# dpeerlab/segger

Hardware: AMD Instinct MI355X
Metric: edges scored/sec (tx->cell) fwd+bwd (higher is better)
Workload: dtype bf16; 1 GPU; C2: single Xenium-scale tile per GPU, 1000000 tx, 10000 nuclei, k=15 kNN (Ett=15000000, Etb=393796, Ep=2435646), training step fwd+bwd+Adam, attention dropout 0.2; parallelism=dp1

## Files before the change

### include/segger_amd.h

```cpp
#ifndef SEGGER_AMD_H
#define SEGGER_AMD_H

#include <stddef.h>
#include <stdint.h>

#ifdef __cplusplus
extern "C" {
#endif

#if defined(__GNUC__) || defined(__clang__)
#pragma GCC visibility push(default)
#endif

#define SEGGER_ABI_VERSION 30

enum segger_status {
  SEGGER_OK = 0,
  SEGGER_EINVAL = -1,
  SEGGER_EUNSUPPORTED = -2,
  SEGGER_EHIP = -3,
  SEGGER_EWORKSPACE = -4
};

enum segger_dtype { SEGGER_F32 = 0, SEGGER_BF16 = 1, SEGGER_F16 = 2 };

typedef void* segger_stream_t;

int segger_abi_version(void);
const char* segger_last_error(void);
// ... 85 lines not shown
  int64_t ld_gxr;
  float* grad_att;
  float* grad_bias;
  void* workspace;
  size_t workspace_bytes;
  const uint8_t* keep_bits_dst;
  const uint8_t* keep_bits_src;
  int32_t src_unique;
  void* zero_rows_out;
  int64_t ld_zero;
  int32_t grad_xl_zeroed;
  int32_t passes;
} segger_gatv2_bwd_args;

size_t segger_gatv2_bwd_workspace_bytes(int64_t n_dst, int32_t heads, int32_t channels);
int segger_gatv2_bwd(const segger_gatv2_bwd_args* args, segger_stream_t stream);
int segger_gatv2_bwd_pair(const segger_gatv2_bwd_args* a, const segger_gatv2_bwd_args* b, segger_stream_t stream);
int segger_dropout_bits(const int32_t* eid, int64_t n_edges, int32_t heads, float dropout_p, const uint64_t* seeds,
                        int32_t n_seeds, const uint64_t* seed_dev, uint8_t* bits, int64_t plane_stride,
                        segger_stream_t stream);
typedef struct segger_bits_job {
  const int32_t* eid;
  int64_t n_edges;
  const uint64_t* seeds;
  int32_t n_seeds;
  int32_t reserved_;
  uint8_t* bits;
  int64_t plane_stride;
} segger_bits_job;
int segger_dropout_bits_many(const segger_bits_job* jobs, int32_t n_jobs, int32_t heads, float dropout_p,
// ... 338 lines not shown
```

### segger_amd/_lib.py

```python
from __future__ import annotations

import ctypes as C
import os
from typing import Optional

import torch

_HERE = os.path.dirname(os.path.abspath(__file__))
LIB_PATH = os.environ.get("SEGGER_AMD_LIB") or os.path.join(_HERE, "libsegger_amd.so")
ABI_VERSION = 30

SEGGER_F32, SEGGER_BF16, SEGGER_F16 = 0, 1, 2
DTYPE_CODE = {torch.float32: SEGGER_F32, torch.bfloat16: SEGGER_BF16, torch.float16: SEGGER_F16}


class SeggerAmdError(RuntimeError):
    pass


c_i64p = C.c_void_p
vp = C.c_void_p


class Csr(C.Structure):
    _fields_ = [("indptr", vp), ("col", vp), ("eid", vp),
# ... 173 lines not shown
class WgradArgs(C.Structure):
    _fields_ = [("dy", vp), ("ld_dy", C.c_int64), ("x", vp), ("ld_x", C.c_int64), ("w_t", vp), ("n_rows", C.c_int64),
                ("m_out", C.c_int32), ("reserved_", C.c_int32), ("grad_w", vp), ("grad_b", vp), ("dx", vp),
                ("ld_dx", C.c_int64), ("workspace", vp), ("workspace_bytes", C.c_size_t)]


EXPORTS = {
    "segger_abi_version": (C.c_int, []),
    "segger_csr_block_tables": (C.c_int, [vp, vp, vp, C.c_int64, C.c_int64, vp, vp, vp, vp, vp]),
    "segger_last_error": (C.c_char_p, []),
    "segger_csr_from_coo_workspace_bytes": (C.c_size_t, [C.c_int64, C.c_int64]),
    "segger_csr_from_coo": (C.c_int, [vp, vp, C.c_int64, C.c_int64, C.c_int64, vp, vp, vp, vp, vp, C.c_size_t, vp]),
    "segger_csr_row_order": (C.c_int, [vp, C.c_int64, C.c_int32, vp, vp]),
    "segger_gatv2_fwd": (C.c_int, [C.POINTER(GatFwdArgs), vp]),
    "segger_gatv2_bwd_workspace_bytes": (C.c_size_t, [C.c_int64, C.c_int32, C.c_int32]),
    "segger_gatv2_bwd": (C.c_int, [C.POINTER(GatBwdArgs), vp]),
    "segger_dropout_bits": (C.c_int, [vp, C.c_int64, C.c_int32, C.c_float, vp, C.c_int32, vp, vp, C.c_int64, vp]),
    "segger_gatv2_has_specialised": (C.c_int, [C.c_int32, C.c_int32]),
    "segger_coo_unique": (C.c_int, [vp, C.c_int64, C.c_int64, vp, vp, vp]),
    "segger_stage": (C.c_int, [C.POINTER(StageSeg), C.c_int32, vp]),
    "segger_adam_step": (C.c_int, [C.POINTER(AdamTensor), C.c_int32, C.c_double, C.c_double, C.c_double, C.c_double, vp]),
    "segger_adam_step_ex": (C.c_int, [C.POINTER(AdamTensor), C.c_int32, C.c_double, C.c_double, C.c_double, C.c_double, C.c_int32, vp, C.c_int64, vp]),
    "segger_adam_step_dev": (C.c_int, [C.POINTER(AdamTensor), C.c_int32, vp, C.c_int32, vp, C.c_int64, vp]),
    "segger_transpose_many": (C.c_int, [C.POINTER(TransposeSeg), C.c_int32, vp]),
    "segger_posmlp_supported": (C.c_int, [C.c_int32, C.c_int32, C.c_int32]),
    "segger_posmlp_fwd": (C.c_int, [vp, vp, vp, vp, C.c_int64, C.c_float, C.c_float, vp, vp, vp, vp, vp, vp, vp, vp, vp,
                                    C.c_int32, C.c_int32, vp]),
    "segger_posmlp_wgrad": (C.c_int, [vp, C.c_int64, vp, C.c_int64, C.c_float, C.c_int32, vp, vp, vp, C.c_size_t, vp]),
    "segger_sample_negatives": (C.c_int, [vp, C.c_int64, C.c_int64, vp, C.c_uint64, vp, vp, vp]),
    "segger_edge_cos_argmax": (C.c_int, [C.POINTER(EdgeArgmaxArgs), vp]),
# ... 158 lines not shown
```

### segger_amd/csrc/gatv2.hip

```cpp
#include "gatv2_launch.h"
#include "draws.h"

namespace segger {

constexpr int kSlabSplits = 128;

__global__ __launch_bounds__(256) void slab_reduce_stage1(const float* __restrict__ slab, int64_t nblocks, int width,
                                                         float* __restrict__ part) {
  __shared__ float sm[4][64];
  const int lane = threadIdx.x & 63, wave = threadIdx.x >> 6;
  const int colx = blockIdx.x * 64 + lane;
  const int64_t per = (nblocks + kSlabSplits - 1) / kSlabSplits;
  const int64_t r0 = (int64_t)blockIdx.y * per;
  const int64_t r1 = r0 + per < nblocks ? r0 + per : nblocks;
  float s = 0.f;
  if (colx < width)
    for (int64_t r = r0 + wave; r < r1; r += 4) s += slab[r * width + colx];
  sm[wave][lane] = s;
  __syncthreads();
  if (wave == 0 && colx < width) part[(int64_t)blockIdx.y * width + colx] = sm[0][lane] + sm[1][lane] + sm[2][lane] + sm[3][lane];
}

__global__ __launch_bounds__(256) void slab_reduce_stage2(const float* __restrict__ part, int width, int hc,
                                                         float* __restrict__ grad_att, float* __restrict__ grad_bias) {
  const int colx = blockIdx.x * 256 + threadIdx.x;
  if (colx >= width) return;
  float t = 0.f;
  for (int r = 0; r < kSlabSplits; ++r) t += part[(int64_t)r * width + colx];
  if (colx < hc) grad_att[colx] = t;
  else if (grad_bias) grad_bias[colx - hc] = t;
}

__global__ __launch_bounds__(256) void zero_rows_kernel(char* __restrict__ base, int64_t pitch, int64_t pieces, int64_t total) {
  const int64_t i = (int64_t)blockIdx.x * 256 + threadIdx.x;
  if (i >= total) return;
  *reinterpret_cast<u32x4*>(base + (i / pieces) * pitch + (i % pieces) * 16) = u32x4{0u, 0u, 0u, 0u};
}

__global__ __launch_bounds__(256) void dropout_bits_kernel(BitsParams p) { dropout_bits_body(p, blockIdx.x); }
__global__ __launch_bounds__(256) void dropout_bits_many_kernel(BitsJobs j) { dropout_bits_body(j.job[blockIdx.y], blockIdx.x); }

namespace {

constexpr double kWavePerRowDegree = 32.0;

// ... 114 lines not shown
                   use_wave_per_row(b->by_dst) && !a->alpha && !b->alpha;
  if (!one) {
    if (!ea) CHECK_RC(launch(Pass::Fwd, pa, a->dtype, a->heads, a->channels, use_wave_per_row(a->by_dst), (hipStream_t)stream));
    if (!eb) CHECK_RC(launch(Pass::Fwd, pb, b->dtype, b->heads, b->channels, use_wave_per_row(b->by_dst), (hipStream_t)stream));
    return SEGGER_OK;
  }
  switch (a->dtype) {
    case SEGGER_F32:  return gatv2_launch_fwd_pair_f32(pa, pb, a->heads, a->channels, (hipStream_t)stream);
    case SEGGER_BF16: return gatv2_launch_fwd_pair_bf16(pa, pb, a->heads, a->channels, (hipStream_t)stream);
    case SEGGER_F16:  return gatv2_launch_fwd_pair_f16(pa, pb, a->heads, a->channels, (hipStream_t)stream);
  }
  set_error("gatv2: unknown dtype %d", a->dtype);
  return SEGGER_EINVAL;
}

extern "C" size_t segger_gatv2_bwd_workspace_bytes(int64_t n_dst, int32_t heads, int32_t channels) {
  if (n_dst <= 0 || heads <= 0 || channels <= 0) return 16;
  const int64_t per = 4 * (int64_t)bwd_row_iters(n_dst);
  const int64_t blocks = (n_dst + per - 1) / per + kNumXcd;
  return (size_t)(blocks + kSlabSplits) * 2 * heads * channels * sizeof(float);
}

namespace {
struct BwdState {
  GatParams p;
  bool direct = false, specialised = false;
  int64_t n_dst = 0, n_src = 0, n_edges = 0;
};

int bwd_prepare(const segger_gatv2_bwd_args* a, BwdState& s) {
  SEGGER_REQUIRE(a != nullptr, "segger_gatv2_bwd: args is NULL");
  SEGGER_REQUIRE(a->heads > 0 && a->channels > 0, "segger_gatv2_bwd: heads/channels must be positive");
  const int hc = a->heads * a->channels;
  const bool specialised = gatv2_has_specialised(a->heads, a->channels);
  g_need_align = specialised;
// ... 12 lines not shown
  if (n_dst > 0) {
    CHECK_RC(check_rows("x_r", a->x_r, a->ld_xr, a->dtype, hc));
    CHECK_RC(check_rows("grad_out", a->grad_out, a->ld_go, a->dtype, hc));
    CHECK_RC(check_rows("pre", a->pre, a->ld_pre, a->dtype, hc));
    CHECK_RC(check_rows("grad_pre", a->grad_pre, a->ld_gp, a->dtype, hc));
    CHECK_RC(check_rows("grad_xr", a->grad_xr, a->ld_gxr, a->dtype, hc));
    SEGGER_REQUIRE(a->lse && a->dsum, "segger_gatv2_bwd: lse / dsum is NULL");
  }
  if (n_src > 0) {
    CHECK_RC(check_rows("x_l", a->x_l, a->ld_xl, a->dtype, hc));
    CHECK_RC(check_rows("grad_xl", a->grad_xl, a->ld_gxl, a->dtype, hc));
  }
  SEGGER_REQUIRE(!(a->dropout_p > 0.f) || n_edges == 0 ||
                     ((a->by_dst.eid || a->keep_bits_dst) && (direct || a->by_src.eid || a->keep_bits_src)),
                 "segger_gatv2_bwd: eid arrays (or keep_bits) are required for dropout");
  const size_t need = segger_gatv2_bwd_workspace_bytes(n_dst, a->heads, a->channels);
  if (a->workspace == nullptr || a->workspace_bytes < need) {
    set_error("segger_gatv2_bwd: workspace %zu < %zu bytes", a->workspace_bytes, need);
    return SEGGER_EWORKSPACE;
  }
  SEGGER_REQUIRE(!a->zero_rows_out || (!direct && specialised),
                 "segger_gatv2_bwd: zero_rows_out needs the two-pass backward of a specialised geometry");
  if (a->zero_rows_out && n_src > 0) CHECK_RC(check_rows("zero_rows_out", a->zero_rows_out, a->ld_zero, a->dtype, hc));

  s.direct = direct; s.specialised = specialised; s.n_dst = n_dst; s.n_src = n_src; s.n_edges = n_edges;
  GatParams& p = s.p;
  p = GatParams{};
  p.xl = a->x_l; p.ld_xl = a->ld_xl; p.xr = a->x_r; p.ld_xr = a->ld_xr;
  p.att = a->att; p.bias = a->bias;
  p.pre = const_cast<void*>(a->pre); p.ld_pre = a->ld_pre; p.lse = const_cast<float*>(a->lse);
  p.gout = a->grad_out; p.ld_go = a->ld_go; p.gpre = a->grad_pre; p.ld_gp = a->ld_gp; p.dsum = a->dsum;
// ... 6 lines not shown

void bwd_dst_params(const segger_gatv2_bwd_args* a, BwdState& s) {
  GatParams& p = s.p;
  p.indptr = a->by_dst.indptr; p.col = a->by_dst.col; p.eid = a->by_dst.eid; p.order = a->by_dst.row_order;
  p.n_rows = s.n_dst; p.n_edges = s.n_edges; p.rows_per_wave_iter = bwd_row_iters(s.n_dst);
  p.bits = a->keep_bits_dst;
  p.direct_gxl = s.direct ? 1 : 0;
  p.zero_rows = nullptr; p.ld_zero = 0;
}

void bwd_src_params(const segger_gatv2_bwd_args* a, BwdState& s) {
  GatParams& p = s.p;
  p.direct_gxl = 0;
  p.indptr = a->by_src.indptr; p.col = a->by_src.col; p.eid = a->by_src.eid; p.order = a->by_src.row_order;
  p.bits = a->keep_bits_src;
  p.n_rows = s.n_src; p.rows_per_wave_iter = 1;
  p.zero_rows = a->zero_rows_out; p.ld_zero = a->ld_zero;
}

int bwd_zero_fill(const segger_gatv2_bwd_args* a, const BwdState& s, hipStream_t stream) {
  const size_t es = elem_size(a->dtype);
  const int64_t pieces = (int64_t)a->heads * a->channels * es / 16, total = s.n_src * pieces;
  hipLaunchKernelGGL(zero_rows_kernel, dim3((unsigned)((total + 255) / 256)), dim3(256), 0, stream,
                     static_cast<char*>(a->grad_xl), (int64_t)a->ld_gxl * (int64_t)es, pieces, total);
  SEGGER_LAUNCH_CHECK("zero_rows_kernel");
  return SEGGER_OK;
}

int bwd_reduce_slab(const segger_gatv2_bwd_args* a, const BwdState& s, hipStream_t stream) {
  if (!s.specialised) return SEGGER_OK;
  const GatParams& p = s.p;
  const int hc = a->heads * a->channels, width = 2 * hc;
  float* part = p.slab + p.nblocks * width;
  if (defer_reduce(ReduceSeg{p.slab, p.nblocks, width, hc, a->grad_att, a->grad_bias, part}, stream)) return SEGGER_OK;
  hipLaunchKernelGGL(slab_reduce_stage1, dim3((width + 63) / 64, kSlabSplits), dim3(256), 0, stream,
                     p.slab, p.nblocks, width, part);
  hipLaunchKernelGGL(slab_reduce_stage2, dim3((width + 255) / 256), dim3(256), 0, stream,
                     part, width, hc, a->grad_att, a->grad_bias);
  SEGGER_LAUNCH_CHECK("slab_reduce kernels");
  return SEGGER_OK;
}

int bwd_no_destinations(const segger_gatv2_bwd_args* a, hipStream_t stream) {
  const int hc = a->heads * a->channels;
  SEGGER_HIP(hipMemsetAsync(a->grad_att, 0, hc * sizeof(float), stream));
  if (a->grad_bias) SEGGER_HIP(hipMemsetAsync(a->grad_bias, 0, hc * sizeof(float), stream));
  return SEGGER_OK;
}

int64_t bwd_pair_max_rows() {
  static const int64_t v = [] {
    const char* e = getenv("SEGGER_BWD_PAIR_MAX_ROWS");
    return e ? (int64_t)atoll(e) : (int64_t)SEGGER_BWD_PAIR_MAX_ROWS;
  }();
  return v;
}
}

extern "C" int segger_gatv2_bwd(const segger_gatv2_bwd_args* a, segger_stream_t stream_) {
  hipStream_t stream = (hipStream_t)stream_;
  BwdState s;
  CHECK_RC(bwd_prepare(a, s));
  SEGGER_REQUIRE(a->passes >= 0 && a->passes <= 3, "segger_gatv2_bwd: passes must be 0 (both), 1 (destination), 2 (source) or 3");
  if (a->passes != 2) {
    bwd_dst_params(a, s);
    if (s.direct && s.n_src > 0 && !a->grad_xl_zeroed) CHECK_RC(bwd_zero_fill(a, s, stream));
    if (s.n_dst > 0) {
      GenericOut gen; gen.grad_att = a->grad_att; gen.grad_bias = a->grad_bias;
      CHECK_RC(launch(Pass::BwdDst, s.p, a->dtype, a->heads, a->channels, use_wave_per_row(a->by_dst), stream, gen));
      if (a->passes != 3) CHECK_RC(bwd_reduce_slab(a, s, stream));
    } else {
      CHECK_RC(bwd_no_destinations(a, stream));
    }
  }
  if (s.direct || a->passes == 1 || a->passes == 3) return SEGGER_OK;
  bwd_src_params(a, s);
  if (s.n_src > 0) CHECK_RC(launch(Pass::BwdSrc, s.p, a->dtype, a->heads, a->channels, use_wave_per_row(a->by_src), stream));
  return SEGGER_OK;
}

extern "C" int segger_gatv2_bwd_pair(const segger_gatv2_bwd_args* a, const segger_gatv2_bwd_args* b, segger_stream_t stream_) {
  hipStream_t stream = (hipStream_t)stream_;
  BwdState sa, sb;
  CHECK_RC(bwd_prepare(a, sa));
  CHECK_RC(bwd_prepare(b, sb));
  const bool zero_by_a = a->zero_rows_out ? (a->zero_rows_out == b->grad_xl && a->ld_zero == b->ld_gxl && b->grad_xl_zeroed)
                                          : !b->grad_xl_zeroed;
  const bool one = !sa.direct && sb.direct && a->dtype == b->dtype && a->heads == b->heads && a->channels == b->channels &&
                   sa.specialised && sa.n_dst > 0 && sa.n_src > 0 && sb.n_dst > 0 && sb.n_src > 0 && sa.n_dst == sb.n_src &&
                   !use_wave_per_row(a->by_dst) && !use_wave_per_row(a->by_src) && use_wave_per_row(b->by_dst) &&
                   zero_by_a && sa.n_src <= bwd_pair_max_rows();
  if (!one) {
    CHECK_RC(segger_gatv2_bwd(a, stream_));
    return segger_gatv2_bwd(b, stream_);
  }
  bwd_dst_params(a, sa);
  sa.p.zero_rows = b->grad_xl; sa.p.ld_zero = b->ld_gxl;
  CHECK_RC(launch(Pass::BwdDst, sa.p, a->dtype, a->heads, a->channels, false, stream));
  CHECK_RC(bwd_reduce_slab(a, sa, stream));
  bwd_src_params(a, sa);
  sa.p.zero_rows = nullptr; sa.p.ld_zero = 0;
  bwd_dst_params(b, sb);
  switch (a->dtype) {
    case SEGGER_F32:  CHECK_RC(gatv2_launch_bwd_src_dst_pair_f32(sa.p, sb.p, a->heads, a->channels, stream)); break;
    case SEGGER_BF16: CHECK_RC(gatv2_launch_bwd_src_dst_pair_bf16(sa.p, sb.p, a->heads, a->channels, stream)); break;
    case SEGGER_F16:  CHECK_RC(gatv2_launch_bwd_src_dst_pair_f16(sa.p, sb.p, a->heads, a->channels, stream)); break;
    default: set_error("gatv2: unknown dtype %d", a->dtype); return SEGGER_EINVAL;
  }
  return bwd_reduce_slab(b, sb, stream);
}

extern "C" int segger_gatv2_has_specialised(int32_t heads, int32_t channels) {
  return gatv2_has_specialised(heads, channels) ? 1 : 0;
}

extern "C" int segger_dropout_bits(const int32_t* eid, int64_t n_edges, int32_t heads, float dropout_p,
                                   const uint64_t* seeds, int32_t n_seeds, const uint64_t* seed_dev, uint8_t* bits,
                                   int64_t plane_stride, segger_stream_t stream) {
  SEGGER_REQUIRE(n_edges >= 0 && heads > 0 && heads <= 8, "segger_dropout_bits: heads must be in 1..8");
  SEGGER_REQUIRE(n_seeds > 0 && n_seeds <= 16 && seeds, "segger_dropout_bits: 1..16 seeds");
  SEGGER_REQUIRE(dropout_p >= 0.f && dropout_p < 1.f, "segger_dropout_bits: dropout_p must be in [0,1)");
  if (n_edges == 0) return SEGGER_OK;
  SEGGER_REQUIRE(eid && bits, "segger_dropout_bits: NULL pointer");
  SEGGER_REQUIRE(plane_stride >= n_edges && plane_stride % 4 == 0 && ((uintptr_t)bits & 3u) == 0,
// ... 61 lines not shown
```

### segger_amd/csrc/gatv2_inst.hip

```cpp
#include "gatv2_launch.h"

#if SEGGER_INST_DTYPE == 0
#define INST_T float
#define INST_TN f32
#elif SEGGER_INST_DTYPE == 1
#define INST_T bf16_t
#define INST_TN bf16
#else
#define INST_T f16_t
#define INST_TN f16
#endif
#if SEGGER_INST_PASS == 0
#define INST_KERNEL gatv2_fwd_kernel
#define INST_PN fwd
#elif SEGGER_INST_PASS == 1
#define INST_KERNEL gatv2_bwd_dst_kernel
#define INST_PN bwd_dst
#else
#define INST_KERNEL gatv2_bwd_src_kernel
#define INST_PN bwd_src
#endif
#define INST_CAT2(a, b, c) gatv2_launch_##a##_##b
#define INST_CAT(a, b) INST_CAT2(a, b, )
#define INST_NAME INST_CAT(INST_PN, INST_TN)
// ... 32 lines not shown
        hipLaunchKernelGGL((gatv2_fwd_lds_kernel<INST_T, H, LPH>), dim3((unsigned)p.nblocks_padded), dim3(256), 0, stream, p); \
        break;                                                                                                         \
      }                                                                                                                \
    }                                                                                                                  \
    hipLaunchKernelGGL((INST_KERNEL<INST_T, H, LPH, WPR>), dim3((unsigned)p.nblocks_padded), dim3(256), 0, stream, p); \
  } while (0)
#else
#define INST_LAUNCH(H, LPH, WPR) \
  hipLaunchKernelGGL((INST_KERNEL<INST_T, H, LPH, WPR>), dim3((unsigned)p.nblocks_padded), dim3(256), 0, stream, p)
#endif

template <int H, int LPH, bool WPR>
int launch_one(GatParams& p, hipStream_t stream) {
  using G = Geo<H, LPH>;
  const int64_t rows_per_wave = WPR ? 1 : G::NG;
  const int iters = (SEGGER_INST_PASS == 1) ? p.rows_per_wave_iter : 1;
  const int64_t rows_per_block = 4 * rows_per_wave * iters;
  p.nblocks = (p.n_rows + rows_per_block - 1) / rows_per_block;
  p.nblocks_padded = pad_to_xcd(p.nblocks);
  if (p.nblocks == 0) return SEGGER_OK;
  if (p.nblocks_padded > 0x7fffffffLL) {
    set_error("gatv2: %lld rows need more than 2^31 blocks", (long long)p.n_rows);
    return SEGGER_EUNSUPPORTED;
  }
  INST_LAUNCH(H, LPH, WPR);
  SEGGER_LAUNCH_CHECK("gatv2 kernel launch");
  return SEGGER_OK;
}

#if SEGGER_INST_PASS == 0
template <int H, int LPH>
// ... 7 lines not shown
  if (grid == 0) return SEGGER_OK;
  if (grid > 0x7fffffffLL) { set_error("gatv2: too many blocks"); return SEGGER_EUNSUPPORTED; }
  hipLaunchKernelGGL((gatv2_fwd_pair_kernel<INST_T, H, LPH>), dim3((unsigned)grid), dim3(256), 0, stream, a, b);
  SEGGER_LAUNCH_CHECK("gatv2 pair launch");
  return SEGGER_OK;
}
#endif

}

#if SEGGER_INST_PASS == 2
namespace {
template <int H, int LPH>
int launch_src_dst_pair(GatParams& a, GatParams& b, hipStream_t stream) {
  using G = Geo<H, LPH>;
  a.nblocks = (a.n_rows + 4 * G::NG - 1) / (4 * G::NG);
  const int64_t per_b = 4 * (int64_t)b.rows_per_wave_iter;
  b.nblocks = (b.n_rows + per_b - 1) / per_b;
  a.nblocks_padded = pad_to_xcd(a.nblocks);
  b.nblocks_padded = pad_to_xcd(b.nblocks);
  const int64_t grid = a.nblocks_padded + b.nblocks_padded;
  if (grid == 0) return SEGGER_OK;
  if (grid > 0x7fffffffLL) { set_error("gatv2: too many blocks"); return SEGGER_EUNSUPPORTED; }
  hipLaunchKernelGGL((gatv2_bwd_src_dst_pair_kernel<INST_T, H, LPH>), dim3((unsigned)grid), dim3(256), 0, stream, a, b);
  SEGGER_LAUNCH_CHECK("gatv2 backward pair launch");
  return SEGGER_OK;
}
}
#define INST_BPAIR_CAT2(a) gatv2_launch_bwd_src_dst_pair_##a
#define INST_BPAIR_CAT(a) INST_BPAIR_CAT2(a)
int INST_BPAIR_CAT(INST_TN)(GatParams& a, GatParams& b, int heads, int channels, hipStream_t stream) {
// ... 33 lines not shown
```

### segger_amd/csrc/gatv2_kernels.h

```cpp
#pragma once
#include "common.h"

namespace segger {

#ifndef SEGGER_FWD_UNROLL
#define SEGGER_FWD_UNROLL 4
#endif
#ifndef SEGGER_FWD_UNROLL_WPR
#define SEGGER_FWD_UNROLL_WPR 2
#endif
#ifndef SEGGER_DST_UNROLL
#define SEGGER_DST_UNROLL 4
#endif
#ifndef SEGGER_SRC_UNROLL
#define SEGGER_SRC_UNROLL 4
#endif

#ifndef SEGGER_FWD_WAVES
#define SEGGER_FWD_WAVES 4
#endif
#ifndef SEGGER_BWD_DST_WAVES
#define SEGGER_BWD_DST_WAVES 3
#endif
#ifndef SEGGER_BWD_SRC_WAVES
// ... 597 lines not shown
        float a_eff = a;
        if constexpr (META != kMetaNone) {
          const bool keep = META == kMetaBits ? (ed[u] & hbit) != 0
                                              : dropout_keep((uint32_t)ed[u], H, h, seed_lo, seed_hi, p.drop_thr);
          da = keep ? da * p.drop_scale : 0.f;
          a_eff = keep ? a * p.drop_scale : 0.f;
        }
        const float de = a * (da - D);
        Sde += de;
        const float nde = -de;
        const f32x2 nde2 = splat(nde);
        f32x2 gx[4];
#pragma unroll
        for (int i = 0; i < 4; ++i) {
          const f32x2 sg = f32x2{sign_mul(nde, nt[i].x), sign_mul(nde, nt[i].y)};
          Pt[i] = pk_fma(nde2, nt[i], Pt[i]);
          Qt[i] = pk_fma(-sg, nt[i], Qt[i]);
          Sg[i] = Sg[i] + sg;
          if constexpr (DIRECT)
            gx[i] = pk_fma(splat(a_eff), g[i], (a1[i] * de + a2[i] * sg) * kLn2);
        }
        if constexpr (DIRECT) {
          if (valid[u] && L.lane_on)
            store_pairs(reinterpret_cast<T*>(gxl_base + (uint64_t)(uint32_t)nbr[u] * ld_gxl), gx);
        }
      }
    };
    if (dropout && p.bits)
      walk_row<GS, WPR, kMetaBits, U>(p.col, p.bits, beg, end, L.lane, L.grp, L.gl, body);
    else if (dropout)
      walk_row<GS, WPR, kMetaEid, U>(p.col, p.eid, beg, end, L.lane, L.grp, L.gl, body);
    else
// ... 3 lines not shown
#pragma unroll
      for (int off = GS; off < 64; off <<= 1) {
        Sde += __shfl_xor(Sde, off, 64);
#pragma unroll
        for (int i = 0; i < 4; ++i) {
          Sg[i].x += __shfl_xor(Sg[i].x, off, 64);
          Sg[i].y += __shfl_xor(Sg[i].y, off, 64);
        }
      }
    }
    if (writer) {
      f32x2 dxr[4];
#pragma unroll
      for (int i = 0; i < 4; ++i) dxr[i] = (a1[i] * Sde + a2[i] * Sg[i]) * kLn2;
      store_pairs(static_cast<T*>(p.gxr) + row * p.ld_gxr + ch0, dxr);
    }
  }

  const float c1 = 0.5f * (1.f + p.slope), c2 = 0.5f * (1.f - p.slope);
  float datt[8], db[8];
#pragma unroll
  for (int i = 0; i < 4; ++i) {
    datt[2 * i] = c1 * Pt[i].x + c2 * Qt[i].x; datt[2 * i + 1] = c1 * Pt[i].y + c2 * Qt[i].y;
    db[2 * i] = dbias[i].x; db[2 * i + 1] = dbias[i].y;
  }
#pragma unroll
  for (int off = GS; off < 64; off <<= 1) {
#pragma unroll
    for (int k = 0; k < 8; ++k) {
      datt[k] += __shfl_xor(datt[k], off, 64);
// ... 7 lines not shown
  __syncthreads();
  for (int i = threadIdx.x; i < 2 * HC; i += 256) {
    const int which = i / HC, c = i % HC;
    p.slab[blk * (2 * HC) + i] = red[0][which][c] + red[1][which][c] + red[2][which][c] + red[3][which][c];
  }
}

template <typename T, int H, int LPH, bool WPR, bool DIRECT>
__global__ __launch_bounds__(256, DIRECT ? 2 : SEGGER_BWD_DST_WAVES) void gatv2_bwd_dst_kernel(GatParams p) {
  gatv2_bwd_dst_body<T, H, LPH, WPR, DIRECT>(p, blockIdx.x);
}

template <typename T, int H, int LPH, bool WPR>
__device__ __forceinline__ void gatv2_bwd_src_body(SEGGER_BODY_PARAM p, int64_t bid) {
  using G = Geo<H, LPH>;
  constexpr int GS = G::GS, NG = G::NG, U = SEGGER_SRC_UNROLL < GS ? SEGGER_SRC_UNROLL : GS;
  const int64_t blk = xcd_remap(bid, p.nblocks_padded, p.nblocks);
  if (blk < 0) return;
  const LaneGeo L = lane_geo<G>();
  const int h = L.h, ch0 = L.ch0;
  const int64_t pos = WPR ? (blk * 4 + L.wave) : ((blk * 4 + L.wave) * NG + L.grp);
  const bool row_ok = pos < p.n_rows;
  const int row = visit_row<WPR>(p.order, pos, row_ok);
  const char* __restrict__ xr_base = static_cast<const char*>(p.xr) + (size_t)ch0 * sizeof(T);
  const char* __restrict__ g_base = static_cast<const char*>(p.gpre) + (size_t)ch0 * sizeof(T);
  const uint32_t ld_xr = (uint32_t)(p.ld_xr * sizeof(T)), ld_gp = (uint32_t)(p.ld_gp * sizeof(T));
  const bool dropout = p.drop_thr != 0;
  uint32_t seed_lo = p.seed_lo, seed_hi = p.seed_hi;
  if (dropout && p.seed_dev) {
    const uint64_t mixed = splitmix64(p.seed_raw + *p.seed_dev);
    seed_lo = (uint32_t)mixed; seed_hi = (uint32_t)(mixed >> 32);
  }

  f32x2 a1[4], na1[4], a2[4], nv[4], acc[4], Sg[4];
#pragma unroll
  for (int i = 0; i < 4; ++i) { nv[i] = splat(0.f); acc[i] = splat(0.f); Sg[i] = splat(0.f); }
  float Sde = 0.f;
  int64_t beg = 0, end = 0;
  if (row_ok) { beg = p.indptr[row]; end = p.indptr[row + 1]; }
  if (__all(beg == end)) {
    if (row_ok && L.lane_on && (!WPR || L.grp == 0)) {
      store_pairs(static_cast<T*>(p.gxl) + row * p.ld_gxl + ch0, acc);
      if (p.zero_rows) store_pairs(static_cast<T*>(p.zero_rows) + row * p.ld_zero + ch0, acc);
    }
    return;
  }
  load_att(p.att, ch0, p.slope, kLog2e, a1, a2);
#pragma unroll
  for (int i = 0; i < 4; ++i) na1[i] = -a1[i];
  if (row_ok) {
    f32x2 v[4];
    load_pairs(static_cast<const T*>(p.xl) + row * p.ld_xl + ch0, v);
#pragma unroll
    for (int i = 0; i < 4; ++i) nv[i] = neg_canon_zero(v[i]);
  }

  const int hbit = 1 << h;
  auto body = [&](auto meta_c, const bool (&valid)[U], const int (&nbr)[U], const int (&ed)[U]) {
    constexpr int META = decltype(meta_c)::value;
    if (!valid[0]) return;
    Raw8<T> rxr[U], rg[U];
    float lse[U], D[U];
#pragma unroll
    for (int u = 0; u < U; ++u) {
      rxr[u].load(row_ptr(xr_base, nbr[u], ld_xr));
      rg[u].load(row_ptr(g_base, nbr[u], ld_gp));
      const float2 ld = *reinterpret_cast<const float2*>(p.dsum + ((int64_t)nbr[u] * H + h) * 2);
      lse[u] = ld.x; D[u] = ld.y;
    }
#pragma unroll
    for (int u = 0; u < U; ++u) {
      f32x2 xr[4], g[4], nt[4];
      rxr[u].get(xr);
      rg[u].get(g);
      f32x2 nda2 = splat(0.f);
#pragma unroll
      for (int i = 0; i < 4; ++i) { nt[i] = nv[i] - xr[i]; nda2 = pk_fma(g[i], nv[i], nda2); }
      const float pl = lane_block_sum<LPH>(logit_partial(nt, na1, a2));
      float da = -lane_block_sum<LPH>(nda2.x + nda2.y);
      const float a = valid[u] ? fast_exp2(pl - lse[u]) : 0.f;
      float a_eff = a;
      if constexpr (META != kMetaNone) {
        const bool keep = META == kMetaBits ? (ed[u] & hbit) != 0
                                            : dropout_keep((uint32_t)ed[u], H, h, seed_lo, seed_hi, p.drop_thr);
        da = keep ? da * p.drop_scale : 0.f;
        a_eff = keep ? a * p.drop_scale : 0.f;
      }
      const float de = a * (da - D[u]);
      Sde += de;
      const f32x2 ae2 = splat(a_eff);
      const float nde = -de;
#pragma unroll
      for (int i = 0; i < 4; ++i) {
        acc[i] = pk_fma(ae2, g[i], acc[i]);
        Sg[i] = Sg[i] + f32x2{sign_mul(nde, nt[i].x), sign_mul(nde, nt[i].y)};
      }
    }
  };
  if (dropout && p.bits)
    walk_row<GS, WPR, kMetaBits, U>(p.col, p.bits, beg, end, L.lane, L.grp, L.gl, body);
  else if (dropout)
    walk_row<GS, WPR, kMetaEid, U>(p.col, p.eid, beg, end, L.lane, L.grp, L.gl, body);
  else
    walk_row<GS, WPR, kMetaNone, U>(p.col, nullptr, beg, end, L.lane, L.grp, L.gl, body);

#pragma unroll
  for (int i = 0; i < 4; ++i) acc[i] = acc[i] + (a1[i] * Sde + a2[i] * Sg[i]) * kLn2;
  if constexpr (WPR) {
#pragma unroll
    for (int off = GS; off < 64; off <<= 1) {
#pragma unroll
      for (int i = 0; i < 4; ++i) {
        acc[i].x += __shfl_xor(acc[i].x, off, 64);
        acc[i].y += __shfl_xor(acc[i].y, off, 64);
      }
    }
  }
  if (row_ok && L.lane_on && (!WPR || L.grp == 0)) {
    store_pairs(static_cast<T*>(p.gxl) + row * p.ld_gxl + ch0, acc);
    if (p.zero_rows) {
      f32x2 z[4];
#pragma unroll
      for (int i = 0; i < 4; ++i) z[i] = splat(0.f);
      store_pairs(static_cast<T*>(p.zero_rows) + row * p.ld_zero + ch0, z);
    }
  }
}

template <typename T, int H, int LPH, bool WPR>
__global__ __launch_bounds__(256, SEGGER_BWD_SRC_WAVES) void gatv2_bwd_src_kernel(GatParams p) {
  gatv2_bwd_src_body<T, H, LPH, WPR>(p, blockIdx.x);
}

template <typename T, int H, int LPH>
__global__ __launch_bounds__(256, 3) void gatv2_bwd_src_dst_pair_kernel(GatParams a, GatParams b) {
  if ((int64_t)blockIdx.x < b.nblocks_padded) gatv2_bwd_dst_body<T, H, LPH, true, true, 2>(b, blockIdx.x);
  else gatv2_bwd_src_body<T, H, LPH, false>(a, (int64_t)blockIdx.x - b.nblocks_padded);
}

}
```

### segger_amd/ops.py

```python
from __future__ import annotations

import ctypes as C
from typing import Optional, Tuple

import torch
from torch import Tensor

from . import _lib
from ._lib import DTYPE_CODE
from . import graph as _graph
from .graph import EdgeCSR, EdgeGraph


def _rows(t: Tensor, width: int, name: str) -> Tuple[int, int]:
    sh = t.shape
    if len(sh) != 2 or sh[1] != width:
        raise ValueError(f"{name}: expected [n, {width}], got {tuple(sh)}")
    st = t.stride()
    if sh[0] > 1:
        if st[1] != 1:
            raise ValueError(f"{name}: last dimension must be contiguous")
        return t.data_ptr(), st[0]
    return t.data_ptr(), max(width, st[0])


import functools
import os


@functools.lru_cache(maxsize=None)
def _has_specialised(heads: int, channels: int) -> bool:
    return bool(_lib.load().segger_gatv2_has_specialised(heads, channels))


@functools.lru_cache(maxsize=4096)
def _gat_bwd_ws_bytes(n_dst: int, heads: int, channels: int) -> int:
    return int(_lib.load().segger_gatv2_bwd_workspace_bytes(n_dst, heads, channels))


@functools.lru_cache(maxsize=4096)
def _wgrad_ws_bytes(n: int, m: int, k: int) -> int:
    return int(_lib.load().segger_linear_wgrad_workspace_bytes(n, m, k))


def _seed_parts(seed):
    if isinstance(seed, tuple):
        value, dev = seed
        return int(value) & 0xFFFFFFFFFFFFFFFF, (None if dev is None else dev.data_ptr())
    return int(seed) & 0xFFFFFFFFFFFFFFFF, None


def _bits_ptr(bits: Tensor, n_edges: int) -> int:
# ... 286 lines not shown
    a.pre, a.ld_pre = _rows(pre, hc, "pre")
    a.lse = lse.data_ptr()
    if scratch is not None:
        grad_pre, dsum = scratch
    else:
        grad_pre = torch.empty((n_dst, hc), dtype=dt, device=dev)
        dsum = torch.empty((n_dst, heads, 2), dtype=torch.float32, device=dev)
    a.passes = int(passes)
    gatv2_bwd_launch.scratch = (grad_pre, dsum)
    a.grad_pre, a.ld_gp = _rows(grad_pre, hc, "grad_pre")
    a.dsum = dsum.data_ptr()
    a.grad_xl, a.ld_gxl = _rows(grad_xl, hc, "grad_xl")
    a.grad_xr, a.ld_gxr = _rows(grad_xr, hc, "grad_xr")
    gparams = torch.empty((2, hc), dtype=torch.float32, device=dev)
    a.grad_att, a.grad_bias = gparams[0].data_ptr(), gparams[1].data_ptr()
    ws_bytes = _gat_bwd_ws_bytes(n_dst, heads, channels)
    ws = torch.empty(ws_bytes, dtype=torch.uint8, device=dev)
    a.workspace, a.workspace_bytes = ws.data_ptr(), ws_bytes
    _defer_keep(ws, gparams)
    return a, gparams, (vecs, grad_out, grad_pre, dsum, ws)


class _GatV2Aggregate(torch.autograd.Function):

    @staticmethod
    def forward(ctx, xl, xr, att, bias, graph: EdgeGraph, heads, channels, apply_gelu,
                negative_slope, dropout_p, seed, want_alpha, keep_bits=None):
        hc = heads * channels
        dev, dt = xl.device, xl.dtype
        n_dst = graph.n_dst
        need_grad = any(ctx.needs_input_grad[:4])
# ... 2321 lines not shown
```

Baseline: 61.80 million edges/s.

## Move attention-gradient accumulation from dst pass to src pass per-row

The destination backward pass in non-direct mode no longer accumulates per-edge att-gradient terms (Pt/Qt FMAs inside the edge loop). Instead it applies a per-row correction, and the source pass computes its own per-row att-gradient contribution, reduces it across the block and writes it to an extra workspace slab. Both slabs are then reduced together. The source pass also gains multi-row-per-wave iteration, and the workspace grows to hold the source slabs. This removes per-edge FMA work from the hot loop. In exchange it adds shuffles, LDS, a sync and slab traffic in the source kernel, plus extra plumbing for accumulate and deferral modes.

```diff
diff --git a/include/segger_amd.h b/include/segger_amd.h
--- a/include/segger_amd.h
+++ b/include/segger_amd.h
@@ -12,7 +12,7 @@
 #pragma GCC visibility push(default)
 #endif
 
-#define SEGGER_ABI_VERSION 30
+#define SEGGER_ABI_VERSION 31
 
 enum segger_status {
   SEGGER_OK = 0,
@@ -128,6 +128,7 @@
 } segger_gatv2_bwd_args;
 
 size_t segger_gatv2_bwd_workspace_bytes(int64_t n_dst, int32_t heads, int32_t channels);
+size_t segger_gatv2_bwd_workspace_bytes_src(int64_t n_dst, int64_t n_src, int32_t heads, int32_t channels);
 int segger_gatv2_bwd(const segger_gatv2_bwd_args* args, segger_stream_t stream);
 int segger_gatv2_bwd_pair(const segger_gatv2_bwd_args* a, const segger_gatv2_bwd_args* b, segger_stream_t stream);
 int segger_dropout_bits(const int32_t* eid, int64_t n_edges, int32_t heads, float dropout_p, const uint64_t* seeds,
diff --git a/segger_amd/_lib.py b/segger_amd/_lib.py
--- a/segger_amd/_lib.py
+++ b/segger_amd/_lib.py
@@ -8,7 +8,7 @@
 
 _HERE = os.path.dirname(os.path.abspath(__file__))
 LIB_PATH = os.environ.get("SEGGER_AMD_LIB") or os.path.join(_HERE, "libsegger_amd.so")
-ABI_VERSION = 30
+ABI_VERSION = 31
 
 SEGGER_F32, SEGGER_BF16, SEGGER_F16 = 0, 1, 2
 DTYPE_CODE = {torch.float32: SEGGER_F32, torch.bfloat16: SEGGER_BF16, torch.float16: SEGGER_F16}
@@ -212,6 +212,7 @@
     "segger_csr_row_order": (C.c_int, [vp, C.c_int64, C.c_int32, vp, vp]),
     "segger_gatv2_fwd": (C.c_int, [C.POINTER(GatFwdArgs), vp]),
     "segger_gatv2_bwd_workspace_bytes": (C.c_size_t, [C.c_int64, C.c_int32, C.c_int32]),
+    "segger_gatv2_bwd_workspace_bytes_src": (C.c_size_t, [C.c_int64, C.c_int64, C.c_int32, C.c_int32]),
     "segger_gatv2_bwd": (C.c_int, [C.POINTER(GatBwdArgs), vp]),
     "segger_dropout_bits": (C.c_int, [vp, C.c_int64, C.c_int32, C.c_float, vp, C.c_int32, vp, vp, C.c_int64, vp]),
     "segger_gatv2_has_specialised": (C.c_int, [C.c_int32, C.c_int32]),
diff --git a/segger_amd/csrc/gatv2.hip b/segger_amd/csrc/gatv2.hip
--- a/segger_amd/csrc/gatv2.hip
+++ b/segger_amd/csrc/gatv2.hip
@@ -22,13 +22,14 @@
 }
 
 __global__ __launch_bounds__(256) void slab_reduce_stage2(const float* __restrict__ part, int width, int hc,
-                                                         float* __restrict__ grad_att, float* __restrict__ grad_bias) {
+                                                         float* __restrict__ grad_att, float* __restrict__ grad_bias,
+                                                         int accumulate) {
   const int colx = blockIdx.x * 256 + threadIdx.x;
   if (colx >= width) return;
   float t = 0.f;
   for (int r = 0; r < kSlabSplits; ++r) t += part[(int64_t)r * width + colx];
-  if (colx < hc) grad_att[colx] = t;
-  else if (grad_bias) grad_bias[colx - hc] = t;
+  if (colx < hc) grad_att[colx] = accumulate ? grad_att[colx] + t : t;
+  else if (grad_bias) grad_bias[colx - hc] = accumulate ? grad_bias[colx - hc] + t : t;
 }
 
 __global__ __launch_bounds__(256) void zero_rows_kernel(char* __restrict__ base, int64_t pitch, int64_t pieces, int64_t total) {
@@ -173,11 +174,22 @@
   return SEGGER_EINVAL;
 }
 
+namespace {
+int64_t bwd_slab_blocks(int64_t n_rows) {
+  if (n_rows <= 0) return 0;
+  const int64_t per = 4 * (int64_t)bwd_row_iters(n_rows);
+  return (n_rows + per - 1) / per + kNumXcd;
+}
+}
+
 extern "C" size_t segger_gatv2_bwd_workspace_bytes(int64_t n_dst, int32_t heads, int32_t channels) {
   if (n_dst <= 0 || heads <= 0 || channels <= 0) return 16;
-  const int64_t per = 4 * (int64_t)bwd_row_iters(n_dst);
-  const int64_t blocks = (n_dst + per - 1) / per + kNumXcd;
-  return (size_t)(blocks + kSlabSplits) * 2 * heads * channels * sizeof(float);
+  return (size_t)(bwd_slab_blocks(n_dst) + kSlabSplits) * 2 * heads * channels * sizeof(float);
+}
+
+extern "C" size_t segger_gatv2_bwd_workspace_bytes_src(int64_t n_dst, int64_t n_src, int32_t heads, int32_t channels) {
+  if (heads <= 0 || channels <= 0 || (n_dst <= 0 && n_src <= 0)) return 16;
+  return (size_t)(bwd_slab_blocks(n_dst) + bwd_slab_blocks(n_src) + kSlabSplits) * 2 * heads * channels * sizeof(float);
 }
 
 namespace {
@@ -220,7 +232,8 @@
   SEGGER_REQUIRE(!(a->dropout_p > 0.f) || n_edges == 0 ||
                      ((a->by_dst.eid || a->keep_bits_dst) && (direct || a->by_src.eid || a->keep_bits_src)),
                  "segger_gatv2_bwd: eid arrays (or keep_bits) are required for dropout");
-  const size_t need = segger_gatv2_bwd_workspace_bytes(n_dst, a->heads, a->channels);
+  const size_t need = direct ? segger_gatv2_bwd_workspace_bytes(n_dst, a->heads, a->channels)
+                              : segger_gatv2_bwd_workspace_bytes_src(n_dst, n_src, a->heads, a->channels);
   if (a->workspace == nullptr || a->workspace_bytes < need) {
     set_error("segger_gatv2_bwd: workspace %zu < %zu bytes", a->workspace_bytes, need);
     return SEGGER_EWORKSPACE;
@@ -257,7 +270,7 @@
   p.direct_gxl = 0;
   p.indptr = a->by_src.indptr; p.col = a->by_src.col; p.eid = a->by_src.eid; p.order = a->by_src.row_order;
   p.bits = a->keep_bits_src;
-  p.n_rows = s.n_src; p.rows_per_wave_iter = 1;
+  p.n_rows = s.n_src; p.rows_per_wave_iter = bwd_row_iters(s.n_src);
   p.zero_rows = a->zero_rows_out; p.ld_zero = a->ld_zero;
 }
 
@@ -270,16 +283,18 @@
   return SEGGER_OK;
 }
 
-int bwd_reduce_slab(const segger_gatv2_bwd_args* a, const BwdState& s, hipStream_t stream) {
+int bwd_reduce_slab(const segger_gatv2_bwd_args* a, const BwdState& s, float* slab, int64_t n_slabs, bool accumulate,
+                    bool may_defer, hipStream_t stream) {
   if (!s.specialised) return SEGGER_OK;
-  const GatParams& p = s.p;
+  if (n_slabs == 0) return SEGGER_OK;
   const int hc = a->heads * a->channels, width = 2 * hc;
-  float* part = p.slab + p.nblocks * width;
-  if (defer_reduce(ReduceSeg{p.slab, p.nblocks, width, hc, a->grad_att, a->grad_bias, part}, stream)) return SEGGER_OK;
+  float* part = slab + n_slabs * width;
+  if (may_defer && !accumulate && defer_reduce(ReduceSeg{slab, n_slabs, width, hc, a->grad_att, a->grad_bias, part}, stream))
+    return SEGGER_OK;
   hipLaunchKernelGGL(slab_reduce_stage1, dim3((width + 63) / 64, kSlabSplits), dim3(256), 0, stream,
-                     p.slab, p.nblocks, width, part);
+                     slab, n_slabs, width, part);
   hipLaunchKernelGGL(slab_reduce_stage2, dim3((width + 255) / 256), dim3(256), 0, stream,
-                     part, width, hc, a->grad_att, a->grad_bias);
+                     part, width, hc, a->grad_att, accumulate ? nullptr : a->grad_bias, accumulate ? 1 : 0);
   SEGGER_LAUNCH_CHECK("slab_reduce kernels");
   return SEGGER_OK;
 }
@@ -305,21 +320,28 @@
   BwdState s;
   CHECK_RC(bwd_prepare(a, s));
   SEGGER_REQUIRE(a->passes >= 0 && a->passes <= 3, "segger_gatv2_bwd: passes must be 0 (both), 1 (destination), 2 (source) or 3");
+  const int width = 2 * a->heads * a->channels;
+  float* const slab = s.p.slab;
+  int64_t dst_slabs = 0;
   if (a->passes != 2) {
     bwd_dst_params(a, s);
     if (s.direct && s.n_src > 0 && !a->grad_xl_zeroed) CHECK_RC(bwd_zero_fill(a, s, stream));
     if (s.n_dst > 0) {
       GenericOut gen; gen.grad_att = a->grad_att; gen.grad_bias = a->grad_bias;
       CHECK_RC(launch(Pass::BwdDst, s.p, a->dtype, a->heads, a->channels, use_wave_per_row(a->by_dst), stream, gen));
-      if (a->passes != 3) CHECK_RC(bwd_reduce_slab(a, s, stream));
+      dst_slabs = s.p.nblocks;
+      if (s.direct || a->passes == 1) CHECK_RC(bwd_reduce_slab(a, s, slab, dst_slabs, false, a->passes == 0, stream));
     } else {
       CHECK_RC(bwd_no_destinations(a, stream));
     }
   }
   if (s.direct || a->passes == 1 || a->passes == 3) return SEGGER_OK;
   bwd_src_params(a, s);
+  s.p.slab = slab + dst_slabs * width;
   if (s.n_src > 0) CHECK_RC(launch(Pass::BwdSrc, s.p, a->dtype, a->heads, a->channels, use_wave_per_row(a->by_src), stream));
-  return SEGGER_OK;
+  const int64_t src_slabs = s.specialised && s.n_src > 0 ? s.p.nblocks : 0;
+  if (a->passes == 2) return bwd_reduce_slab(a, s, s.p.slab, src_slabs, true, false, stream);
+  return bwd_reduce_slab(a, s, slab, dst_slabs + src_slabs, false, true, stream);
 }
 
 extern "C" int segger_gatv2_bwd_pair(const segger_gatv2_bwd_args* a, const segger_gatv2_bwd_args* b, segger_stream_t stream_) {
@@ -340,9 +362,11 @@
   bwd_dst_params(a, sa);
   sa.p.zero_rows = b->grad_xl; sa.p.ld_zero = b->ld_gxl;
   CHECK_RC(launch(Pass::BwdDst, sa.p, a->dtype, a->heads, a->channels, false, stream));
-  CHECK_RC(bwd_reduce_slab(a, sa, stream));
+  float* const slab_a = sa.p.slab;
+  const int64_t dst_slabs_a = sa.p.nblocks;
   bwd_src_params(a, sa);
   sa.p.zero_rows = nullptr; sa.p.ld_zero = 0;
+  sa.p.slab = slab_a + dst_slabs_a * 2 * a->heads * a->channels;
   bwd_dst_params(b, sb);
   switch (a->dtype) {
     case SEGGER_F32:  CHECK_RC(gatv2_launch_bwd_src_dst_pair_f32(sa.p, sb.p, a->heads, a->channels, stream)); break;
@@ -350,7 +374,8 @@
     case SEGGER_F16:  CHECK_RC(gatv2_launch_bwd_src_dst_pair_f16(sa.p, sb.p, a->heads, a->channels, stream)); break;
     default: set_error("gatv2: unknown dtype %d", a->dtype); return SEGGER_EINVAL;
   }
-  return bwd_reduce_slab(b, sb, stream);
+  CHECK_RC(bwd_reduce_slab(a, sa, slab_a, dst_slabs_a + sa.p.nblocks, false, true, stream));
+  return bwd_reduce_slab(b, sb, sb.p.slab, sb.p.nblocks, false, true, stream);
 }
 
 extern "C" int segger_gatv2_has_specialised(int32_t heads, int32_t channels) {
diff --git a/segger_amd/csrc/gatv2_inst.hip b/segger_amd/csrc/gatv2_inst.hip
--- a/segger_amd/csrc/gatv2_inst.hip
+++ b/segger_amd/csrc/gatv2_inst.hip
@@ -70,7 +70,7 @@
 int launch_one(GatParams& p, hipStream_t stream) {
   using G = Geo<H, LPH>;
   const int64_t rows_per_wave = WPR ? 1 : G::NG;
-  const int iters = (SEGGER_INST_PASS == 1) ? p.rows_per_wave_iter : 1;
+  const int iters = (SEGGER_INST_PASS != 0) ? p.rows_per_wave_iter : 1;
   const int64_t rows_per_block = 4 * rows_per_wave * iters;
   p.nblocks = (p.n_rows + rows_per_block - 1) / rows_per_block;
   p.nblocks_padded = pad_to_xcd(p.nblocks);
@@ -108,7 +108,8 @@
 template <int H, int LPH>
 int launch_src_dst_pair(GatParams& a, GatParams& b, hipStream_t stream) {
   using G = Geo<H, LPH>;
-  a.nblocks = (a.n_rows + 4 * G::NG - 1) / (4 * G::NG);
+  const int64_t per_a = 4 * G::NG * (int64_t)a.rows_per_wave_iter;
+  a.nblocks = (a.n_rows + per_a - 1) / per_a;
   const int64_t per_b = 4 * (int64_t)b.rows_per_wave_iter;
   b.nblocks = (b.n_rows + per_b - 1) / per_b;
   a.nblocks_padded = pad_to_xcd(a.nblocks);
diff --git a/segger_amd/csrc/gatv2_kernels.h b/segger_amd/csrc/gatv2_kernels.h
--- a/segger_amd/csrc/gatv2_kernels.h
+++ b/segger_amd/csrc/gatv2_kernels.h
@@ -635,8 +635,10 @@
 #pragma unroll
         for (int i = 0; i < 4; ++i) {
           const f32x2 sg = f32x2{sign_mul(nde, nt[i].x), sign_mul(nde, nt[i].y)};
-          Pt[i] = pk_fma(nde2, nt[i], Pt[i]);
-          Qt[i] = pk_fma(-sg, nt[i], Qt[i]);
+          if constexpr (DIRECT) {
+            Pt[i] = pk_fma(nde2, nt[i], Pt[i]);
+            Qt[i] = pk_fma(-sg, nt[i], Qt[i]);
+          }
           Sg[i] = Sg[i] + sg;
           if constexpr (DIRECT)
             gx[i] = pk_fma(splat(a_eff), g[i], (a1[i] * de + a2[i] * sg) * kLn2);
@@ -670,6 +672,10 @@
 #pragma unroll
       for (int i = 0; i < 4; ++i) dxr[i] = (a1[i] * Sde + a2[i] * Sg[i]) * kLn2;
       store_pairs(static_cast<T*>(p.gxr) + row * p.ld_gxr + ch0, dxr);
+      if constexpr (!DIRECT) {
+#pragma unroll
+        for (int i = 0; i < 4; ++i) { Pt[i] = pk_fma(splat(-Sde), nxr[i], Pt[i]); Qt[i] = pk_fma(-Sg[i], nxr[i], Qt[i]); }
+      }
     }
   }
 
@@ -707,16 +713,14 @@
 template <typename T, int H, int LPH, bool WPR>
 __device__ __forceinline__ void gatv2_bwd_src_body(SEGGER_BODY_PARAM p, int64_t bid) {
   using G = Geo<H, LPH>;
-  constexpr int GS = G::GS, NG = G::NG, U = SEGGER_SRC_UNROLL < GS ? SEGGER_SRC_UNROLL : GS;
+  constexpr int GS = G::GS, NG = G::NG, U = SEGGER_SRC_UNROLL < GS ? SEGGER_SRC_UNROLL : GS, HC = G::HC;
+  __shared__ float red[4][HC];
   const int64_t blk = xcd_remap(bid, p.nblocks_padded, p.nblocks);
   if (blk < 0) return;
   const LaneGeo L = lane_geo<G>();
-  const int h = L.h, ch0 = L.ch0;
-  const int64_t pos = WPR ? (blk * 4 + L.wave) : ((blk * 4 + L.wave) * NG + L.grp);
-  const bool row_ok = pos < p.n_rows;
-  const int row = visit_row<WPR>(p.order, pos, row_ok);
-  const char* __restrict__ xr_base = static_cast<const char*>(p.xr) + (size_t)ch0 * sizeof(T);
-  const char* __restrict__ g_base = static_cast<const char*>(p.gpre) + (size_t)ch0 * sizeof(T);
+  const int h = L.h;
+  const char* __restrict__ xr_base = static_cast<const char*>(p.xr) + (size_t)L.ch0 * sizeof(T);
+  const char* __restrict__ g_base = static_cast<const char*>(p.gpre) + (size_t)L.ch0 * sizeof(T);
   const uint32_t ld_xr = (uint32_t)(p.ld_xr * sizeof(T)), ld_gp = (uint32_t)(p.ld_gp * sizeof(T));
   const bool dropout = p.drop_thr != 0;
   uint32_t seed_lo = p.seed_lo, seed_hi = p.seed_hi;
@@ -724,100 +728,135 @@
     const uint64_t mixed = splitmix64(p.seed_raw + *p.seed_dev);
     seed_lo = (uint32_t)mixed; seed_hi = (uint32_t)(mixed >> 32);
   }
-
-  f32x2 a1[4], na1[4], a2[4], nv[4], acc[4], Sg[4];
-#pragma unroll
-  for (int i = 0; i < 4; ++i) { nv[i] = splat(0.f); acc[i] = splat(0.f); Sg[i] = splat(0.f); }
-  float Sde = 0.f;
-  int64_t beg = 0, end = 0;
-  if (row_ok) { beg = p.indptr[row]; end = p.indptr[row + 1]; }
-  if (__all(beg == end)) {
+  constexpr int RPW = WPR ? 1 : NG;
+  const float c1 = 0.5f * (1.f + p.slope), c2 = 0.5f * (1.f - p.slope);
+
+  f32x2 a1[4], na1[4], a2[4], gatt[4];
+  load_att(p.att, L.ch0, p.slope, kLog2e, a1, a2);
+#pragma unroll
+  for (int i = 0; i < 4; ++i) { na1[i] = -a1[i]; gatt[i] = splat(0.f); }
+
+#pragma unroll 1
+  for (int it = 0; it < p.rows_per_wave_iter; ++it) {
+    const int64_t rbase = ((blk * (int64_t)p.rows_per_wave_iter + it) * 4 + L.wave) * RPW;
+    if (rbase >= p.n_rows) break;
+    const int64_t pos = rbase + (WPR ? 0 : L.grp);
+    const bool row_ok = pos < p.n_rows;
+    const int row = visit_row<WPR>(p.order, pos, row_ok);
+    int ch0r = L.ch0;
+    asm volatile("" : "+v"(ch0r));
+    const int ch0 = ch0r;
+
+    f32x2 nv[4], acc[4], Sg[4];
+#pragma unroll
+    for (int i = 0; i < 4; ++i) { nv[i] = splat(0.f); acc[i] = splat(0.f); Sg[i] = splat(0.f); }
+    float Sde = 0.f;
+    int64_t beg = 0, end = 0;
+    if (row_ok) { beg = p.indptr[row]; end = p.indptr[row + 1]; }
+    if (__all(beg == end)) {
+      if (row_ok && L.lane_on && (!WPR || L.grp == 0)) {
+        store_pairs(static_cast<T*>(p.gxl) + row * p.ld_gxl + ch0, acc);
+        if (p.zero_rows) store_pairs(static_cast<T*>(p.zero_rows) + row * p.ld_zero + ch0, acc);
+      }
+      continue;
+    }
+    if (row_ok) {
+      f32x2 v[4];
+      load_pairs(static_cast<const T*>(p.xl) + row * p.ld_xl + ch0, v);
+#pragma unroll
+      for (int i = 0; i < 4; ++i) nv[i] = neg_canon_zero(v[i]);
+    }
+
+    const int hbit = 1 << h;
+    auto body = [&](auto meta_c, const bool (&valid)[U], const int (&nbr)[U], const int (&ed)[U]) {
+      constexpr int META = decltype(meta_c)::value;
+      if (!valid[0]) return;
+      Raw8<T> rxr[U], rg[U];
+      float lse[U], D[U];
+#pragma unroll
+      for (int u = 0; u < U; ++u) {
+        rxr[u].load(row_ptr(xr_base, nbr[u], ld_xr));
+        rg[u].load(row_ptr(g_base, nbr[u], ld_gp));
+        const float2 ld = *reinterpret_cast<const float2*>(p.dsum + ((int64_t)nbr[u] * H + h) * 2);
+        lse[u] = ld.x; D[u] = ld.y;
+      }
+#pragma unroll
+      for (int u = 0; u < U; ++u) {
+        f32x2 xr[4], g[4], nt[4];
+        rxr[u].get(xr);
+        rg[u].get(g);
+        f32x2 nda2 = splat(0.f);
+#pragma unroll
+        for (int i = 0; i < 4; ++i) { nt[i] = nv[i] - xr[i]; nda2 = pk_fma(g[i], nv[i], nda2); }
+        const float pl = lane_block_sum<LPH>(logit_partial(nt, na1, a2));
+        float da = -lane_block_sum<LPH>(nda2.x + nda2.y);
+        const float a = valid[u] ? fast_exp2(pl - lse[u]) : 0.f;
+        float a_eff = a;
+        if constexpr (META != kMetaNone) {
+          const bool keep = META == kMetaBits ? (ed[u] & hbit) != 0
+                                              : dropout_keep((uint32_t)ed[u], H, h, seed_lo, seed_hi, p.drop_thr);
+          da = keep ? da * p.drop_scale : 0.f;
+          a_eff = keep ? a * p.drop_scale : 0.f;
+        }
+        const float de = a * (da - D[u]);
+        Sde += de;
+        const f32x2 ae2 = splat(a_eff);
+        const float nde = -de;
+#pragma unroll
+        for (int i = 0; i < 4; ++i) {
+          acc[i] = pk_fma(ae2, g[i], acc[i]);
+          Sg[i] = Sg[i] + f32x2{sign_mul(nde, nt[i].x), sign_mul(nde, nt[i].y)};
+        }
+      }
+    };
+    if (dropout && p.bits)
+      walk_row<GS, WPR, kMetaBits, U>(p.col, p.bits, beg, end, L.lane, L.grp, L.gl, body);
+    else if (dropout)
+      walk_row<GS, WPR, kMetaEid, U>(p.col, p.eid, beg, end, L.lane, L.grp, L.gl, body);
+    else
+      walk_row<GS, WPR, kMetaNone, U>(p.col, nullptr, beg, end, L.lane, L.grp, L.gl, body);
+
+#pragma unroll
+    for (int i = 0; i < 4; ++i) {
+      acc[i] = acc[i] + (a1[i] * Sde + a2[i] * Sg[i]) * kLn2;
+      gatt[i] = pk_fma(nv[i], pk_fma(splat(-c2), Sg[i], splat(-c1 * Sde)), gatt[i]);
+    }
+    if constexpr (WPR) {
+#pragma unroll
+      for (int off = GS; off < 64; off <<= 1) {
+#pragma unroll
+        for (int i = 0; i < 4; ++i) {
+          acc[i].x += __shfl_xor(acc[i].x, off, 64);
+          acc[i].y += __shfl_xor(acc[i].y, off, 64);
+        }
+      }
+    }
     if (row_ok && L.lane_on && (!WPR || L.grp == 0)) {
       store_pairs(static_cast<T*>(p.gxl) + row * p.ld_gxl + ch0, acc);
-      if (p.zero_rows) store_pairs(static_cast<T*>(p.zero_rows) + row * p.ld_zero + ch0, acc);
-    }
-    return;
-  }
-  load_att(p.att, ch0, p.slope, kLog2e, a1, a2);
-#pragma unroll
-  for (int i = 0; i < 4; ++i) na1[i] = -a1[i];
-  if (row_ok) {
-    f32x2 v[4];
-    load_pairs(static_cast<const T*>(p.xl) + row * p.ld_xl + ch0, v);
-#pragma unroll
-    for (int i = 0; i < 4; ++i) nv[i] = neg_canon_zero(v[i]);
-  }
-
-  const int hbit = 1 << h;
-  auto body = [&](auto meta_c, const bool (&valid)[U], const int (&nbr)[U], const int (&ed)[U]) {
-    constexpr int META = decltype(meta_c)::value;
-    if (!valid[0]) return;
-    Raw8<T> rxr[U], rg[U];
-    float lse[U], D[U];
-#pragma unroll
-    for (int u = 0; u < U; ++u) {
-      rxr[u].load(row_ptr(xr_base, nbr[u], ld_xr));
-      rg[u].load(row_ptr(g_base, nbr[u], ld_gp));
-      const float2 ld = *reinterpret_cast<const float2*>(p.dsum + ((int64_t)nbr[u] * H + h) * 2);
-      lse[u] = ld.x; D[u] = ld.y;
-    }
-#pragma unroll
-    for (int u = 0; u < U; ++u) {
-      f32x2 xr[4], g[4], nt[4];
-      rxr[u].get(xr);
-      rg[u].get(g);
-      f32x2 nda2 = splat(0.f);
-#pragma unroll
-      for (int i = 0; i < 4; ++i) { nt[i] = nv[i] - xr[i]; nda2 = pk_fma(g[i], nv[i], nda2); }
-      const float pl = lane_block_sum<LPH>(logit_partial(nt, na1, a2));
-      float da = -lane_block_sum<LPH>(nda2.x + nda2.y);
-      const float a = valid[u] ? fast_exp2(pl - lse[u]) : 0.f;
-      float a_eff = a;
-      if constexpr (META != kMetaNone) {
-        const bool keep = META == kMetaBits ? (ed[u] & hbit) != 0
-                                            : dropout_keep((uint32_t)ed[u], H, h, seed_lo, seed_hi, p.drop_thr);
-        da = keep ? da * p.drop_scale : 0.f;
-        a_eff = keep ? a * p.drop_scale : 0.f;
-      }
-      const float de = a * (da - D[u]);
-      Sde += de;
-      const f32x2 ae2 = splat(a_eff);
-      const float nde = -de;
-#pragma unroll
-      for (int i = 0; i < 4; ++i) {
-        acc[i] = pk_fma(ae2, g[i], acc[i]);
-        Sg[i] = Sg[i] + f32x2{sign_mul(nde, nt[i].x), sign_mul(nde, nt[i].y)};
-      }
-    }
-  };
-  if (dropout && p.bits)
-    walk_row<GS, WPR, kMetaBits, U>(p.col, p.bits, beg, end, L.lane, L.grp, L.gl, body);
-  else if (dropout)
-    walk_row<GS, WPR, kMetaEid, U>(p.col, p.eid, beg, end, L.lane, L.grp, L.gl, body);
-  else
-    walk_row<GS, WPR, kMetaNone, U>(p.col, nullptr, beg, end, L.lane, L.grp, L.gl, body);
-
-#pragma unroll
-  for (int i = 0; i < 4; ++i) acc[i] = acc[i] + (a1[i] * Sde + a2[i] * Sg[i]) * kLn2;
-  if constexpr (WPR) {
-#pragma unroll
-    for (int off = GS; off < 64; off <<= 1) {
-#pragma unroll
-      for (int i = 0; i < 4; ++i) {
-        acc[i].x += __shfl_xor(acc[i].x, off, 64);
-        acc[i].y += __shfl_xor(acc[i].y, off, 64);
-      }
-    }
-  }
-  if (row_ok && L.lane_on && (!WPR || L.grp == 0)) {
-    store_pairs(static_cast<T*>(p.gxl) + row * p.ld_gxl + ch0, acc);
-    if (p.zero_rows) {
-      f32x2 z[4];
-#pragma unroll
-      for (int i = 0; i < 4; ++i) z[i] = splat(0.f);
-      store_pairs(static_cast<T*>(p.zero_rows) + row * p.ld_zero + ch0, z);
-    }
-  }
+      if (p.zero_rows) {
+        f32x2 z[4];
+#pragma unroll
+        for (int i = 0; i < 4; ++i) z[i] = splat(0.f);
+        store_pairs(static_cast<T*>(p.zero_rows) + row * p.ld_zero + ch0, z);
+      }
+    }
+  }
+
+  float datt[8];
+#pragma unroll
+  for (int i = 0; i < 4; ++i) { datt[2 * i] = gatt[i].x; datt[2 * i + 1] = gatt[i].y; }
+#pragma unroll
+  for (int off = GS; off < 64; off <<= 1) {
+#pragma unroll
+    for (int k = 0; k < 8; ++k) datt[k] += __shfl_xor(datt[k], off, 64);
+  }
+  if (L.grp == 0 && L.lane_on) {
+#pragma unroll
+    for (int k = 0; k < 8; ++k) red[L.wave][L.ch0 + k] = datt[k];
+  }
+  __syncthreads();
+  for (int i = threadIdx.x; i < 2 * HC; i += 256)
+    p.slab[blk * (2 * HC) + i] = i < HC ? red[0][i] + red[1][i] + red[2][i] + red[3][i] : 0.f;
 }
 
 template <typename T, int H, int LPH, bool WPR>
diff --git a/segger_amd/ops.py b/segger_amd/ops.py
--- a/segger_amd/ops.py
+++ b/segger_amd/ops.py
@@ -34,8 +34,8 @@
 
 
 @functools.lru_cache(maxsize=4096)
-def _gat_bwd_ws_bytes(n_dst: int, heads: int, channels: int) -> int:
-    return int(_lib.load().segger_gatv2_bwd_workspace_bytes(n_dst, heads, channels))
+def _gat_bwd_ws_bytes(n_dst: int, n_src: int, heads: int, channels: int) -> int:
+    return int(_lib.load().segger_gatv2_bwd_workspace_bytes_src(n_dst, n_src, heads, channels))
 
 
 @functools.lru_cache(maxsize=4096)
@@ -352,7 +352,7 @@
     a.grad_xr, a.ld_gxr = _rows(grad_xr, hc, "grad_xr")
     gparams = torch.empty((2, hc), dtype=torch.float32, device=dev)
     a.grad_att, a.grad_bias = gparams[0].data_ptr(), gparams[1].data_ptr()
-    ws_bytes = _gat_bwd_ws_bytes(n_dst, heads, channels)
+    ws_bytes = _gat_bwd_ws_bytes(n_dst, g.n_src, heads, channels)
     ws = torch.empty(ws_bytes, dtype=torch.uint8, device=dev)
     a.workspace, a.workspace_bytes = ws.data_ptr(), ws_bytes
     _defer_keep(ws, gparams)
```

Result: slower. 56.09 million edges/s, median of 2 (-9.2%).
